# sdbds/ACE-Step-1.5-for-windows

Measured on AMD Instinct MI355X. Metric: songs/sec (30 s audio @ 27 DiT steps, CFG 7 + APG, batch 8 in total, DiT + VAE decode), higher is better.
Workload: dtype bf16; 1 GPU; acestep-5Hz base DiT (24L/2048d, 1.575B params, random init) + Oobleck decoder, 30 s audio (T=750), 27 steps, CFG 7 (2x8 sequences/forward on rank 0), L=769, 8 songs per request over 1 GPU(s); infer_steps=27, batch_per_gpu=8, batch_rank0=8, global_batch=8, parallelism=dp1, tiny=False, sampler_chains_per_gpu=1, batch_dependent_bits=True

## Files before the change

### ace-step-1.5-for-windows_amd/csrc/common.h

```cpp
#pragma once
#include <hip/hip_runtime.h>
#include <stdint.h>
#include <string>

namespace ace355 {

void set_error(const std::string& msg);
int hip_fail(hipError_t e, const char* what, const char* file, int line);

#define ACE_HIP(expr)                                                          \
    do {                                                                       \
        hipError_t _e = (expr);                                                \
        if (_e != hipSuccess) return ::ace355::hip_fail(_e, #expr, __FILE__, __LINE__); \
    } while (0)

#define ACE_CHECK(cond, msg)                                  \
    do {                                                      \
        if (!(cond)) {                                        \
            ::ace355::set_error(std::string("invalid argument: ") + (msg)); \
            return 1;                                         \
        }                                                     \
    } while (0)

#define ACE_LAUNCH_CHECK() ACE_HIP(hipGetLastError())
// ... 182 lines not shown
int launch_latent_check(const float* x, long n, int* flags_dev, hipStream_t s);
int launch_zero_u64(unsigned long long* p, long n, hipStream_t s);

enum PackMode { PACK_ROWS = 0, PACK_ROWS_IL32 = 1, PACK_CONV_IN = 2, PACK_CONVT_OUT = 3, PACK_ROWS_HEADPAIR = 4 };
__host__ __device__ __forceinline__ long pack_row(int mode, long r, long dst_row0, int p0) {
    if (mode == PACK_ROWS_IL32) return dst_row0 + (r >> 5) * 64 + p0 * 32 + (r & 31);
    if (mode == PACK_ROWS_HEADPAIR) {
        const long d = r & 127;
        return dst_row0 + (r - d) + (d < 64 ? 2 * d : 2 * (d - 64) + 1);
    }
    return dst_row0 + r;
}
int launch_pack(const void* src, int src_dtype, void* dst, int dst_is_bf16, int mode, long rows, long cols, long dst_ld,
                long dst_row0, int p0, int p1, hipStream_t s);

struct ConvArgs {
    const bf16_t* x; long x_batch_stride; int L_in; int Cin;
    long x_shift; long x_valid;
    const bf16_t* w;
    const float* bias;
    const float* alpha; const float* beta;
    const bf16_t* res; long res_batch_stride;
    void* y; long y_batch_stride;
    int B, M, N, taps, dil, center;
    long y_shift; long y_valid;
    int out_mode;
    int n_real;
    long ncl_ld; long ncl_off; int ncl_m_lo; int ncl_m_hi;
    int wide_ok;
    int clk_probe;
    const bf16_t* w2; const float* bias2; const float* alpha2; const float* beta2;
    const float* osnake_a; const float* osnake_b;
    int ras_tm; int ras_tn;
};
int launch_conv(const ConvArgs& a, hipStream_t s);
int launch_ncl_to_nlc(const float* z, bf16_t* out, int B, int C, int T, hipStream_t s);

constexpr int LORA_TILE_ROWS = 64, LORA_TILE_COLS = 128;
struct LoraTermDev {
    const bf16_t* A;
    const bf16_t* B;
    int rank;
    float scale;
};
struct LoraTargetDev {
    bf16_t* dst;
    const bf16_t* src;
    long ld;
    long row0;
    int mode, p0;
    int rows, cols;
    int tile0, tiles_n;
    int term0, nterms;
};
int launch_lora_merge(const LoraTargetDev* targets_dev, int n_targets, int total_tiles, const LoraTermDev* terms_dev, hipStream_t s);
int launch_lora_read(const bf16_t* w, long ld, int mode, long row0, int p0, long rows, long cols, void* dst, int dst_is_bf16,
                     hipStream_t s);

constexpr int XATTN_MAX_HEADS = 64;
struct XattnArgs {
    const bf16_t* q; long q_seq_stride; int q_ld;
    unsigned long long k_tab[64]; int k_ld;
    float* out;
    int N, Sq, Skv, Hq, Hkv, n_heads;
    int heads[XATTN_MAX_HEADS];
    float scale;
// ... 5 lines not shown
```

### ace-step-1.5-for-windows_amd/csrc/conv.hip

```cpp
#include <stdio.h>
#include <stdlib.h>

#include "common.h"


namespace ace355 {

namespace {

__device__ __forceinline__ int lds_off(int row, int slot) { return row * 128 + ((slot ^ ((row >> 1) & 7)) << 4); }

__device__ unsigned long long g_conv_probe[8];

typedef unsigned int u32x4 __attribute__((ext_vector_type(4)));
__device__ __forceinline__ u32x4 ld_u32x4(const void* p) {
    return *reinterpret_cast<const __attribute__((address_space(1))) u32x4*>(reinterpret_cast<uintptr_t>(p));
}

__device__ __forceinline__ void conv_glds16_v(const void* vptr, unsigned lds_addr) {
    unsigned keep;
    asm volatile("s_mov_b32 %0, m0\n\ts_mov_b32 m0, %2\n\ts_nop 0\n\tglobal_load_lds_dwordx4 %1, off\n\ts_mov_b32 m0, %0"
                 : "=&s"(keep)
                 : "v"(vptr), "s"(lds_addr)
                 : "memory");
}

constexpr int HALO_MAX = 64;

__device__ __forceinline__ void conv_glds16(unsigned voff, const void* sbase, unsigned lds_addr) {
    unsigned keep;
    asm volatile("s_mov_b32 %0, m0\n\ts_mov_b32 m0, %3\n\ts_nop 0\n\tglobal_load_lds_dwordx4 %1, %2\n\ts_mov_b32 m0, %0"
                 : "=&s"(keep)
                 : "v"(voff), "s"(sbase), "s"(lds_addr)
                 : "memory");
}

__device__ __forceinline__ bf16x8 frag_kperm(const char* base, int row, int q, int h) {
    const uint2 lo = *reinterpret_cast<const uint2*>(base + lds_off(row, 2 * q) + 8 * h);
    const uint2 hi = *reinterpret_cast<const uint2*>(base + lds_off(row, 2 * q + 1) + 8 * h);
    return as_bf16x8(make_uint4(lo.x, lo.y, hi.x, hi.y));
}

template <int BN, int TM, int WS = 0>
__global__ __launch_bounds__(TM * 2, TM / 64) void conv_kernel(ConvArgs a) {
    static_assert(TM == 128 || (TM == 256 && BN == 128), "tile shapes");
    static_assert(WS == 0 || (TM == 256 && BN == 128), "the 32 x 128 wave shape belongs to the fused 8-wave form");
    constexpr int NTHR = TM * 2;
    constexpr int WIN_MAX = TM + HALO_MAX;
    constexpr int MT = WS ? 1 : ((BN == 128) ? 2 : 1);
    constexpr int NT = WS ? 4 : ((BN == 128) ? 2 : 1);
    constexpr int WCH = BN * 8 / NTHR;
    constexpr int FUSE_LDS = (BN == 128 && TM == 128) ? (BN * 128 + 2048) : (WS ? 2048 : 0);
    __shared__ __attribute__((aligned(16))) char smem[WIN_MAX * 128 + 2 * BN * 128 + FUSE_LDS];
    char* As = smem;
    char* Wbase = smem + WIN_MAX * 128;

    const int tid = threadIdx.x, lane = tid & 63, wave = tid >> 6;
    const int lq = lane & 31, half = lane >> 5;
    const int wm = WS ? wave : ((BN == 128) ? (wave >> 1) : wave);
    const int wn = WS ? 0 : ((BN == 128) ? (wave & 1) : 0);
    int bx = blockIdx.x, by = blockIdx.y;
    if (a.ras_tn > 1) {
        const int L = blockIdx.x, tn = a.ras_tn, full = (a.ras_tm >> 3) << 3;
        if (L < full * tn) {
            const int q = L >> 3;
            by = q % tn;
            bx = (q / tn) * 8 + (L & 7);
        } else {
            const int l2 = L - full * tn;
            by = l2 % tn;
            bx = full + l2 / tn;
        }
    }
    const int m0 = bx * TM, n0 = by * BN, b = blockIdx.z;
    const int Cin = a.Cin, taps = a.taps, dil = a.dil;
    const int win_rows = TM + (taps - 1) * dil;
    const int x_row0 = m0 - a.center * dil;
    const bf16_t* xb = a.x + (long)b * a.x_batch_stride;
    const long wrow = (long)taps * Cin;

    f32x16 acc[MT][NT];
#pragma unroll
    for (int i = 0; i < MT; ++i)
#pragma unroll
        for (int j = 0; j < NT; ++j)
#pragma unroll
            for (int r = 0; r < 16; ++r) acc[i][j][r] = 0.f;

    const int sslot = tid & 7;
    constexpr int NWV = NTHR / 64;
    static_assert(WCH * NWV * 8 == BN, "pieces split evenly over the waves");
    unsigned w_voff[WCH];
    int wst[WCH];
#pragma unroll
    for (int i = 0; i < WCH; ++i) {
        const int prow = 8 * (wave + NWV * i) + (lane >> 3);
        const int ls = (lane & 7) ^ ((prow >> 1) & 7);
        w_voff[i] = (unsigned)(((long)min(n0 + prow, a.N - 1) * wrow + ls * 8) * 2);
        wst[i] = lds_off((tid >> 3) + (NTHR / 8) * i, sslot);
    }
    const unsigned wlds0 = (unsigned)(uintptr_t)Wbase + (unsigned)__builtin_amdgcn_readfirstlane(wave) * 1024u;
    auto w_piece = [&](int i, int tap, int ci0, int buf) {
        const bf16_t* sb = a.w + (long)tap * Cin + ci0;
        const unsigned lb = (unsigned)__builtin_amdgcn_readfirstlane((int)(wlds0 + (unsigned)buf * (BN * 128)));
        conv_glds16(w_voff[i], sb, lb + (unsigned)i * (NWV * 1024));
    };
    auto w_issue = [&](int tap, int ci0, int buf) {
// ... 88 lines not shown
        for (int i = 0; i < WLD; ++i) {
            const int c = tid + i * NTHR;
            if (c < win_rows * 8) *reinterpret_cast<u32x4*>(As + st0 + i * (NTHR / 8) * 128) = wv[i];
        }
    };
    const bool probe = a.clk_probe && blockIdx.x == gridDim.x / 2 && blockIdx.y == 0 && blockIdx.z == 0 && __builtin_amdgcn_readfirstlane(wave) == 0;
    unsigned long long p_t0 = 0, p_w0 = 0, p_stage = 0, p_taps = 0, p_mark = 0;
    if (probe) p_t0 = clock64(), p_w0 = wall_clock64();
    constexpr bool FPIPE = (TM == 128);
    if (PREFETCH) { win_load(0); if (PARPRE) par_load(0); }
    for (int ci0 = 0; ci0 < Cin; ci0 += 64) {
        if (probe) p_mark = clock64();
        if (!PREFETCH) win_load(ci0);
        __syncthreads();
        if (PREFETCH) __builtin_amdgcn_s_waitcnt(0x0F70);
        w_issue(0, ci0, 0);
        win_store(ci0);
        asm volatile("s_waitcnt vmcnt(0)" ::: "memory");
        __syncthreads();
        if (PREFETCH && ci0 + 64 < Cin) { win_load(ci0 + 64); if (PARPRE) par_load(ci0 + 64); }
        if (probe) { const unsigned long long t = clock64(); p_stage += t - p_mark; p_mark = t; }

#pragma unroll 1
        for (int tap = 0; tap < taps; ++tap) {
            const bool more = (tap + 1) < taps;
            if (more) w_issue(tap + 1, ci0, (tap + 1) & 1);
            if constexpr (FUSE_LDS != 0) {
                if (a.w2 && ci0 + 64 >= Cin) {
                    constexpr int PT_OFF = (WS ? 2 : 3) * BN * 128;
                    if constexpr (WS == 0) {
                        const unsigned w2b = (unsigned)(uintptr_t)(Wbase + 2 * BN * 128) + (unsigned)__builtin_amdgcn_readfirstlane(wave) * 1024u;
                        if (tap >= 1 && tap <= WCH) w2_piece(tap - 1, 0, w2b);
                    }
                    if (tap == 5 && __builtin_amdgcn_readfirstlane(wave) < 2) {
                        const float* src = (wave == 0) ? (lane < 32 ? (a.bias ? a.bias : a.alpha2) : a.alpha2)
                                                       : (lane < 32 ? a.beta2 : (a.bias2 ? a.bias2 : a.beta2));
                        conv_glds16_v(src + 4 * (lane & 31), (unsigned)(uintptr_t)(Wbase + PT_OFF) + (unsigned)__builtin_amdgcn_readfirstlane(wave) * 1024u);
                    }
                    if (!more) {
                        const unsigned ring = wlds0 + (unsigned)((tap + 1) & 1) * (BN * 128);
#pragma unroll
                        for (int i = 0; i < WCH; ++i) w2_piece(i, WS ? 0 : 1, ring);
                    }
                }
            }
            const char* Ws = Wbase + (tap & 1) * (BN * 128);
            const int arow = wm * (MT * 32) + tap * dil + lq;
            if constexpr (FPIPE) {
                bf16x8 fa[2][MT], fw[2][NT];
                auto frag = [&](int kk, int sl) {
#pragma unroll
                    for (int i = 0; i < MT; ++i)
                        fa[sl][i] = as_bf16x8(*reinterpret_cast<const uint4*>(As + lds_off(arow + i * 32, kk * 2 + half)));
#pragma unroll
                    for (int j = 0; j < NT; ++j)
                        fw[sl][j] = as_bf16x8(*reinterpret_cast<const uint4*>(Ws + lds_off(wn * (NT * 32) + j * 32 + lq, kk * 2 + half)));
                };
                frag(0, 0);
#pragma unroll
                for (int kk = 0; kk < 4; ++kk) {
                    if (kk < 3) frag(kk + 1, (kk + 1) & 1);
                    __builtin_amdgcn_sched_barrier(0);
#pragma unroll
                    for (int i = 0; i < MT; ++i)
#pragma unroll
                        for (int j = 0; j < NT; ++j) acc[i][j] = mfma32(fw[kk & 1][j], fa[kk & 1][i], acc[i][j]);
                    __builtin_amdgcn_sched_barrier(0);
                }
            } else {
#pragma unroll
                for (int kk = 0; kk < 4; ++kk) {
                    bf16x8 fa[MT], fw[NT];
#pragma unroll
                    for (int i = 0; i < MT; ++i)
                        fa[i] = as_bf16x8(*reinterpret_cast<const uint4*>(As + lds_off(arow + i * 32, kk * 2 + half)));
#pragma unroll
                    for (int j = 0; j < NT; ++j)
                        fw[j] = as_bf16x8(*reinterpret_cast<const uint4*>(Ws + lds_off(wn * (NT * 32) + j * 32 + lq, kk * 2 + half)));
#pragma unroll
                    for (int i = 0; i < MT; ++i)
#pragma unroll
                        for (int j = 0; j < NT; ++j) acc[i][j] = mfma32(fw[j], fa[i], acc[i][j]);
                }
            }
            if (more) {
                asm volatile("s_waitcnt vmcnt(0)" ::: "memory");
                __syncthreads();
            }
        }
        if (probe) p_taps += clock64() - p_mark;
    }
    const bool full = (m0 + TM <= a.M) && (n0 + BN <= a.N) &&
                      ((long)m0 * a.N + n0 + a.y_shift >= 0) && ((long)(m0 + TM - 1) * a.N + n0 + BN - 1 + a.y_shift < a.y_valid);
    const bool wide = BN == 128 && a.out_mode == 0 && full && a.wide_ok;
    const int mw0 = m0 + wm * (MT * 32), nw0 = n0 + wn * (NT * 32);
    const int row_l = lane >> 2, c4 = lane & 3;
    u32x4 bl[NT], bh[NT];
    u32x4 rv[2][MT * 2];
    const bool has_res = (TM == 128 || WS == 1) && a.res != nullptr;
    auto res_load = [&](int j, u32x4 (&r)[MT * 2]) {
        const long rcol = (long)b * a.res_batch_stride + nw0 + j * 32 + c4 * 8 + a.y_shift;
#pragma unroll
        for (int t = 0; t < MT * 2; ++t) r[t] = ld_u32x4(a.res + rcol + (long)(mw0 + t * 16 + row_l) * a.N);
    };
    auto epi_pre = [&](const float* eb) {
#pragma unroll
        for (int j = 0; j < NT; ++j) {
            bl[j] = u32x4{0u, 0u, 0u, 0u};
            bh[j] = u32x4{0u, 0u, 0u, 0u};
        }
        if (eb && WS == 0) {
#pragma unroll
            for (int j = 0; j < NT; ++j) {
                bl[j] = ld_u32x4(eb + nw0 + j * 32 + c4 * 8);
                bh[j] = ld_u32x4(eb + nw0 + j * 32 + c4 * 8 + 4);
            }
        }
        if (has_res) res_load(0, rv[0]);
    };
    bool epi_pre_done = false;
    const float* epi_bias = a.bias;
    bool bias_in_lds = false;
    if constexpr (WS == 1) {
        if (a.w2) {
            epi_bias = a.bias2;
            bias_in_lds = a.bias2 != nullptr;
            const float b7s = a.bias ? 1.f : 0.f;
            const char* W2c0 = Wbase + (taps & 1) * (BN * 128);
            const char* W2c1 = Wbase + ((taps + 1) & 1) * (BN * 128);
            const char* Pt = Wbase + 2 * BN * 128;
            __syncthreads();
            {
                const unsigned ring = wlds0 + (unsigned)(taps & 1 ? 0 : 1) * (BN * 128);
#pragma unroll
                for (int i = 0; i < WCH; ++i) w2_piece(i, 1, ring);
            }
// ... 86 lines not shown
                    const char* Ap = A2 + (k8 >> 2) * 16384;
                    const char* Wp = (k8 >> 2) ? W2c1 : W2c0;
                    const int kk = k8 & 3;
#pragma unroll
                    for (int i = 0; i < MT; ++i) fa[sl][i] = frag_kperm(Ap, wm * (MT * 32) + i * 32 + lq, kk, half);
#pragma unroll
                    for (int j = 0; j < NT; ++j) fw[sl][j] = frag_kperm(Wp, wn * (NT * 32) + j * 32 + lq, kk, half);
                };
                frag2(0, 0);
#pragma unroll
                for (int k8 = 0; k8 < 8; ++k8) {
                    if (k8 < 7) frag2(k8 + 1, (k8 + 1) & 1);
                    __builtin_amdgcn_sched_barrier(0);
#pragma unroll
                    for (int i = 0; i < MT; ++i)
#pragma unroll
                        for (int j = 0; j < NT; ++j) acc[i][j] = mfma32(fw[k8 & 1][j], fa[k8 & 1][i], acc[i][j]);
                    __builtin_amdgcn_sched_barrier(0);
                }
            }
        }
    }
    const unsigned long long p_e0 = probe ? clock64() : 0ull;
    auto probe_done = [&]() {
        if (!probe) return;
        __builtin_amdgcn_s_waitcnt(0x0F70);
        const unsigned long long t = clock64();
        g_conv_probe[0] = t - p_t0, g_conv_probe[1] = p_stage, g_conv_probe[2] = p_taps, g_conv_probe[3] = t - p_e0;
        g_conv_probe[4] = wall_clock64() - p_w0, g_conv_probe[5] = (unsigned long long)(Cin / 64);
    };

    if (wide) {
        if (!epi_pre_done) epi_pre(epi_bias);
        __syncthreads();
        char* stg = smem + wave * (MT * 32 * 128);
#pragma unroll
        for (int j = 0; j < NT; ++j) {
#pragma unroll
            for (int i = 0; i < MT; ++i)
#pragma unroll
                for (int g = 0; g < 4; ++g) {
                    float4 v;
                    v.x = acc[i][j][4 * g + 0]; v.y = acc[i][j][4 * g + 1]; v.z = acc[i][j][4 * g + 2]; v.w = acc[i][j][4 * g + 3];
                    const int row = i * 32 + lq, slot = 2 * g + half;
                    *reinterpret_cast<float4*>(stg + row * 128 + ((slot ^ (row & 7)) << 4)) = v;
                }
            if (has_res && j + 1 < NT) res_load(j + 1, rv[(j + 1) & 1]);
            u32x4 oa[2], ob[2];
            if (a.osnake_a) {
#pragma unroll
                for (int q = 0; q < 2; ++q) {
                    oa[q] = ld_u32x4(a.osnake_a + nw0 + j * 32 + c4 * 8 + 4 * q);
                    ob[q] = ld_u32x4(a.osnake_b + nw0 + j * 32 + c4 * 8 + 4 * q);
                }
            }
            const long col = (long)b * a.y_batch_stride + nw0 + j * 32 + c4 * 8 + a.y_shift;
            if constexpr (WS == 1) {
                if (bias_in_lds) {
                    const char* pb = Wbase + 2 * BN * 128 + 1536 + (nw0 + j * 32 + c4 * 8) * 4;
                    bl[j] = *reinterpret_cast<const u32x4*>(pb);
                    bh[j] = *reinterpret_cast<const u32x4*>(pb + 16);
                } else if (epi_bias) {
                    bl[j] = ld_u32x4(epi_bias + nw0 + j * 32 + c4 * 8);
                    bh[j] = ld_u32x4(epi_bias + nw0 + j * 32 + c4 * 8 + 4);
                }
            }
            const float bias[8] = {__uint_as_float(bl[j][0]), __uint_as_float(bl[j][1]), __uint_as_float(bl[j][2]), __uint_as_float(bl[j][3]),
                                   __uint_as_float(bh[j][0]), __uint_as_float(bh[j][1]), __uint_as_float(bh[j][2]), __uint_as_float(bh[j][3])};
#pragma unroll
            for (int t = 0; t < MT * 2; ++t) {
                const int row = t * 16 + row_l;
                const float4 lo = *reinterpret_cast<const float4*>(stg + row * 128 + (((2 * c4) ^ (row & 7)) << 4));
                const float4 hi = *reinterpret_cast<const float4*>(stg + row * 128 + (((2 * c4 + 1) ^ (row & 7)) << 4));
                float v[8] = {lo.x + bias[0], lo.y + bias[1], lo.z + bias[2], lo.w + bias[3],
                              hi.x + bias[4], hi.y + bias[5], hi.z + bias[6], hi.w + bias[7]};
                if (has_res) {
                    const u32x4 r = rv[j & 1][t];
#pragma unroll
                    for (int e2 = 0; e2 < 4; ++e2) { v[2 * e2] += bf_lo(r[e2]); v[2 * e2 + 1] += bf_hi(r[e2]); }
                }
                if (a.osnake_a) {
#pragma unroll
                    for (int e = 0; e < 8; ++e) {
                        const float sn = __sinf(__uint_as_float(oa[e >> 2][e & 3]) * v[e]);
                        v[e] = v[e] + __uint_as_float(ob[e >> 2][e & 3]) * sn * sn;
                    }
                }
                u32x4 pk = {pack_bf2(v[0], v[1]), pack_bf2(v[2], v[3]), pack_bf2(v[4], v[5]), pack_bf2(v[6], v[7])};
                *reinterpret_cast<u32x4*>(reinterpret_cast<bf16_t*>(a.y) + col + (long)(mw0 + row) * a.N) = pk;
            }
        }
        probe_done();
        return;
    }
#pragma unroll
    for (int i = 0; i < MT; ++i) {
        const int m = mw0 + i * 32 + lq;
        if (m >= a.M) continue;
#pragma unroll
        for (int j = 0; j < NT; ++j)
#pragma unroll
            for (int r = 0; r < 16; ++r) {
                const int n = nw0 + j * 32 + 8 * (r >> 2) + 4 * half + (r & 3);
                if (n >= a.N) continue;
                float v = acc[i][j][r] + (epi_bias ? epi_bias[n] : 0.f);
                if (a.out_mode == 0) {
                    const long flat = (long)m * a.N + n + a.y_shift;
                    if (flat < 0 || flat >= a.y_valid) continue;
                    if (a.res) v += bf2f(a.res[(long)b * a.res_batch_stride + flat]);
                    if (a.osnake_a) {
                        const float sn = __sinf(a.osnake_a[n] * v);
                        v = v + a.osnake_b[n] * sn * sn;
                    }
                    reinterpret_cast<bf16_t*>(a.y)[(long)b * a.y_batch_stride + flat] = f2bf(v);
                } else {
                    if (n < a.n_real) {
                        if (a.ncl_ld == 0) reinterpret_cast<float*>(a.y)[(long)b * a.y_batch_stride + (long)n * a.M + m] = v;
                        else if (m >= a.ncl_m_lo && m < a.ncl_m_hi)
                            reinterpret_cast<float*>(a.y)[(long)b * a.y_batch_stride + (long)n * a.ncl_ld + a.ncl_off + (m - a.ncl_m_lo)] = v;
                    }
                }
            }
    }
}

__global__ void ncl_to_nlc_kernel(const float* __restrict__ z, bf16_t* __restrict__ out, int C, int T, long total) {
    const long i = (long)blockIdx.x * blockDim.x + threadIdx.x;
    if (i >= total) return;
    const int c = (int)(i % C);
    const long bt = i / C;
    const int t = (int)(bt % T);
    const long b = bt / T;
    out[i] = f2bf(z[(b * C + c) * T + t]);
}

}

int launch_conv(const ConvArgs& a, hipStream_t s) {
    ACE_CHECK(a.Cin % 64 == 0, "conv: Cin must be a multiple of 64");
    ACE_CHECK(a.taps >= 1 && (a.taps - 1) * a.dil <= HALO_MAX && a.dil >= 1, "conv: window too large");
    ACE_CHECK(a.B > 0 && a.M > 0 && a.N > 0, "conv: empty problem");
    ACE_CHECK((long)a.N * a.taps * a.Cin * 2 < (1L << 32) && (reinterpret_cast<uintptr_t>(a.w) & 15) == 0,
              "conv: the weight tensor must be 16-byte aligned and smaller than 4 GB (32-bit DMA offsets)");
    ACE_CHECK(a.x_valid ? (a.x_shift % 8 == 0 && a.x_valid % 8 == 0) : a.x_shift == 0, "conv: x_shift / x_valid must be multiples of 8 (and x_shift needs x_valid)");
    ACE_CHECK(!a.w2 || (a.Cin == 128 && a.N == 128 && a.taps == 7 && !a.x_valid && a.out_mode == 0 && a.alpha2 && a.beta2 &&
                        (reinterpret_cast<uintptr_t>(a.alpha2) & 15) == 0 && (reinterpret_cast<uintptr_t>(a.beta2) & 15) == 0 &&
                        (reinterpret_cast<uintptr_t>(a.bias) & 15) == 0 && (reinterpret_cast<uintptr_t>(a.w2) & 15) == 0),
              "conv: the fused k = 1 stage needs Cin = N = 128, a plain conv and 16-byte aligned vectors");
    ACE_CHECK(!a.osnake_a == !a.osnake_b && (!a.osnake_a || a.out_mode == 0), "conv: the producer-side Snake needs both parameter vectors and the bf16 output");
    ConvArgs aw = a;
    {
        auto al16 = [](const void* p) { return (reinterpret_cast<uintptr_t>(p) & 15) == 0; };
        aw.wide_ok = a.out_mode == 0 && al16(a.y) && al16(a.res) && al16(a.bias) && al16(a.bias2) && al16(a.osnake_a) && al16(a.osnake_b) &&
                     (a.N % 8) == 0 && (a.y_shift % 8) == 0 &&
                     (a.y_batch_stride % 8) == 0 && (a.res_batch_stride % 8) == 0;
    }
    static int tm_env = -1, clk_env = -1, ras_env = -1;
    if (ras_env < 0) {
        const char* e = getenv("ACE355_CONV_RAS");
        ras_env = e ? atoi(e) : 1;
    }
    if (clk_env < 0) {
        const char* e = getenv("ACE355_CONV_CLK");
        clk_env = e ? atoi(e) : 0;
    }
    aw.clk_probe = clk_env;
    if (tm_env < 0) {
        const char* e = getenv("ACE355_CONV_TM");
        tm_env = e ? atoi(e) : 0;
    }
    if (a.N >= 128 || a.N % 128 == 0) {
        const long wgs128 = (long)((a.M + 127) / 128) * ((a.N + 127) / 128) * a.B;
        const bool tall_k = a.Cin >= 128 && a.taps >= 3 && wgs128 >= 1400;
        const bool tall_t = a.taps == 2 && a.Cin >= 128 && !a.alpha && !a.x_valid && wgs128 >= 1500;
        const bool tall = !a.w2 && !a.res && (tm_env ? tm_env == 256 : (tall_k || tall_t));
        const int tm_rows = tall ? 256 : 128;
        dim3 grid((a.M + tm_rows - 1) / tm_rows, (a.N + 127) / 128, a.B);
        aw.ras_tm = aw.ras_tn = 0;
        if (ras_env && grid.y > 1 && (long)grid.x * grid.y < (1L << 31)) {
            aw.ras_tm = (int)grid.x, aw.ras_tn = (int)grid.y;
            grid = dim3(grid.x * grid.y, 1, a.B);
        }
        static int f8_env = -2;
        if (f8_env == -2) {
            const char* e = getenv("ACE355_CONV_F8");
            f8_env = e ? atoi(e) : -1;
        }
        const bool f8 = a.w2 && (f8_env >= 0 ? f8_env != 0 : wgs128 >= 1400);
        if (f8) {
            dim3 g8((a.M + 255) / 256, 1, a.B);
            aw.ras_tm = aw.ras_tn = 0;
            hipLaunchKernelGGL((conv_kernel<128, 256, 1>), g8, dim3(512), 0, s, aw);
        } else
        if (tall) hipLaunchKernelGGL((conv_kernel<128, 256>), grid, dim3(512), 0, s, aw);
        else hipLaunchKernelGGL((conv_kernel<128, 128>), grid, dim3(256), 0, s, aw);
    } else {
        aw.ras_tm = aw.ras_tn = 0;
        dim3 grid((a.M + 127) / 128, (a.N + 31) / 32, a.B);
        hipLaunchKernelGGL((conv_kernel<32, 128>), grid, dim3(256), 0, s, aw);
    }
    ACE_LAUNCH_CHECK();
    if (aw.clk_probe) {
        ACE_HIP(hipStreamSynchronize(s));
        unsigned long long h[8];
        ACE_HIP(hipMemcpyFromSymbol(h, HIP_SYMBOL(g_conv_probe), sizeof(h)));
        fprintf(stderr, "[conv clk] Cin=%d N=%d taps=%d dil=%d M=%d: total %llu cyc = stage %llu + taps %llu + epilogue %llu (+%llu other), wall %.2f us, %llu chunks\n",
                a.Cin, a.N, a.taps, a.dil, a.M, h[0], h[1], h[2], h[3], h[0] - h[1] - h[2] - h[3], h[4] / 100.0, h[5]);
    }
    return 0;
}

int launch_ncl_to_nlc(const float* z, bf16_t* out, int B, int C, int T, hipStream_t s) {
    const long total = (long)B * C * T;
    hipLaunchKernelGGL(ncl_to_nlc_kernel, dim3((unsigned)((total + 255) / 256)), dim3(256), 0, s, z, out, C, T, total);
    ACE_LAUNCH_CHECK();
    return 0;
}

}
```

### ace-step-1.5-for-windows_amd/csrc/vae.hip

```cpp
#include <math.h>
#include <string.h>

#include <algorithm>
#include <map>
#include <string>
#include <vector>

#include "../../include/ace355.h"
#include "common.h"

using namespace ace355;

namespace {

struct ConvW {
    bf16_t* w = nullptr;
    float* bias = nullptr;
    int N = 0, taps = 0, Cin = 0;
};
struct SnakeP {
    float* ea = nullptr;
    float* ib = nullptr;
};
struct ResUnitW {
// ... 300 lines not shown
    c->bias = b->p;
    ACE_LAUNCH_CHECK();
    return 0;
}

int build_snake_tiled(ace355_vae* h, const std::string& base, int C, int reps, SnakeP* sp) {
    SnakeP one;
    int rc = build_snake(h, base, C, &one);
    if (rc) return rc;
    if ((rc = valloc(h, &sp->ea, (size_t)C * reps))) return rc;
    if ((rc = valloc(h, &sp->ib, (size_t)C * reps))) return rc;
    hipLaunchKernelGGL(tile_bias_kernel, dim3((C * reps + 255) / 256), dim3(256), 0, 0, one.ea, sp->ea, C, reps);
    hipLaunchKernelGGL(tile_bias_kernel, dim3((C * reps + 255) / 256), dim3(256), 0, 0, one.ib, sp->ib, C, reps);
    ACE_LAUNCH_CHECK();
    return 0;
}

int build_res_unit(ace355_vae* h, const std::string& r, int C, int dil, ResUnitW* R) {
    int rc;
    R->dil = dil;
    if ((rc = build_snake(h, r + ".snake1", C, &R->s1))) return rc;
    if ((rc = build_conv(h, r + ".conv1", C, C, 7, true, &R->c1))) return rc;
    if ((rc = build_snake(h, r + ".snake2", C, &R->s2))) return rc;
    return build_conv(h, r + ".conv2", C, C, 1, true, &R->c2);
}

int run_conv(ace355_vae* h, const ConvArgs& a, hipStream_t s) {
    hipEvent_t e0 = nullptr, e1 = nullptr;
    if (h->profile) {
        hipEventCreate(&e0); hipEventCreate(&e1);
        hipEventRecord(e0, s);
        h->flops += 2.0 * a.B * (double)a.M * (a.out_mode == 1 ? a.n_real : a.N) * a.taps * a.Cin;
        if (a.w2) h->flops += 2.0 * a.B * (double)a.M * a.N * a.N;
        h->launches++;
    }
    int rc = launch_conv(a, s);
    if (h->profile) {
        hipEventRecord(e1, s);
        h->ev.push_back({e0, e1});
    }
    return rc;
}

}

extern "C" {

int ace355_vae_create(const ace355_vae_config* cfg, ace355_vae** out) {
    ACE_CHECK(cfg && out, "vae_create: null argument");
    ACE_CHECK(cfg->num_blocks > 0 && cfg->num_blocks <= ACE355_MAX_BLOCKS, "vae_create: num_blocks");
    ACE_CHECK(cfg->decoder_input_channels % 64 == 0 && cfg->decoder_channels % 64 == 0, "vae_create: channels must be multiples of 64");
    ACE_CHECK(cfg->audio_channels >= 1 && cfg->audio_channels <= 32, "vae_create: audio_channels");
    ace355_vae* h = new ace355_vae();
    h->cfg = *cfg;
    h->hop = 1;
    for (int i = 0; i < cfg->num_blocks; ++i) {
        ACE_CHECK(cfg->upsampling_ratios[i] >= 1 && cfg->channel_multiples[i] >= 1, "vae_create: ratios/multiples");
        h->hop *= cfg->upsampling_ratios[i];
    }
    if (const char* e = getenv("ACE355_VAE_BUDGET_MB")) { const long mb = atol(e); if (mb > 0) h->decode_budget = (size_t)mb << 20; }
    *out = h;
    return ACE355_OK;
}

void ace355_vae_destroy(ace355_vae* h) {
    if (!h) return;
// ... 92 lines not shown
        }
        if ((rc = build_snake(h, "encoder.snake1", EH * cm[nb], &h->e_s_out))) return rc;
        if ((rc = build_conv(h, "encoder.conv2", EH, EH * cm[nb], 3, true, &h->e_conv2))) return rc;
    }
    ACE_HIP(hipDeviceSynchronize());
    for (auto& kv : h->raw) {
        const std::string& k = kv.first;
        const bool keep = k.size() > 5 && k.compare(k.size() - 5, 5, ".bias") == 0;
        if (!keep && kv.second.p) { hipFree(kv.second.p); kv.second.p = nullptr; }
    }
    if (!h->scratch) ACE_HIP(hipMalloc((void**)&h->scratch, 1024));
    h->finalized = true;
    return ACE355_OK;
}

int ace355_vae_hop(const ace355_vae* h) { return h ? h->hop : 0; }

static int episnake_on() {
    static int on = -1;
    if (on < 0) {
        const char* e = getenv("ACE355_VAE_EPISNAKE");
        on = e ? atoi(e) : 1;
    }
    return on;
}
static bool unit_fused(int C) {
    static int fuse = -1;
    if (fuse < 0) {
        const char* e = getenv("ACE355_CONV_FUSE_RU");
        fuse = e ? atoi(e) : 1;
    }
    return fuse && C == 128;
}

static void stage_push(std::vector<ace355_vae_stage_info>& v, int kind, int block, int unit, int channels, int flags, int src, int res,
                       int dil, long rows) {
    ace355_vae_stage_info si;
    si.kind = kind; si.block = block; si.unit = unit; si.channels = channels; si.flags = flags; si.src = src; si.res = res;
    si.dilation = dil; si.rows = rows;
    v.push_back(si);
}
static void stage_push_unit(std::vector<ace355_vae_stage_info>& v, int block, int unit, int C, int dil, long rows, bool epi, bool out_snake) {
    const int in = (int)v.size() - 1;
    const int osn = out_snake ? ACE355_VAE_FLAG_OUT_SNAKE : 0;
    if (unit_fused(C)) {
        stage_push(v, ACE355_VAE_STAGE_UNIT, block, unit, C, ACE355_VAE_FLAG_FUSED | ACE355_VAE_FLAG_IN_SNAKE | osn, in, in, dil, rows);
        return;
    }
    stage_push(v, ACE355_VAE_STAGE_UNIT_K7, block, unit, C, ACE355_VAE_FLAG_IN_SNAKE | (epi ? ACE355_VAE_FLAG_OUT_SNAKE : 0), in, -1, dil, rows);
    stage_push(v, ACE355_VAE_STAGE_UNIT_K1, block, unit, C, (epi ? 0 : ACE355_VAE_FLAG_IN_SNAKE) | osn, in + 1, in, 1, rows);
}
static int stage_list(const ace355_vae* h, int enc, long T, std::vector<ace355_vae_stage_info>& v) {
    v.clear();
    const ace355_vae_config& c = h->cfg;
    if (!enc) {
        const bool epi = episnake_on() != 0 && !h->blocks.empty();
        stage_push(v, ACE355_VAE_STAGE_INPUT, -1, -1, c.decoder_input_channels, 0, -1, -1, 1, T);
        stage_push(v, ACE355_VAE_STAGE_CONV_IN, -1, -1, h->conv1.N, epi ? ACE355_VAE_FLAG_OUT_SNAKE : 0, 0, -1, 1, T);
        long L = T;
        for (size_t bi = 0; bi < h->blocks.size(); ++bi) {
            const BlockW& Bk = h->blocks[bi];
            L = (L - 1) * Bk.stride - 2 * Bk.pad + 2 * Bk.stride;
            stage_push(v, ACE355_VAE_STAGE_CONVT, (int)bi, -1, Bk.cout, epi ? 0 : ACE355_VAE_FLAG_IN_SNAKE, (int)v.size() - 1, -1, 1, L);
            for (int j = 0; j < 3; ++j) stage_push_unit(v, (int)bi, j, Bk.cout, Bk.ru[j].dil, L, epi, epi && j == 2);
        }
        return 0;
// ... 19 lines not shown
static int tap_stage(ace355_vae* h, int enc, int kind, const void* p, int B, hipStream_t s) {
    if (h->tap_stages.empty()) return 0;
    const int k = h->tap_next++;
    ACE_CHECK(k < (int)h->tap_stages.size() && h->tap_stages[k].kind == kind, "vae tap: the stage list and the launch sequence disagree");
    auto it = h->taps[enc].find(k);
    if (it == h->taps[enc].end()) return 0;
    const ace355_vae_stage_info& si = h->tap_stages[k];
    const size_t bytes = (size_t)B * si.rows * si.channels * ((si.flags & ACE355_VAE_FLAG_F32_NCL) ? 4 : 2);
    ACE_CHECK(bytes <= it->second.second, "vae tap: the destination is smaller than the stage");
    ACE_HIP(hipMemcpyAsync(it->second.first, p, bytes, hipMemcpyDeviceToDevice, s));
    return 0;
}
static int tap_begin(ace355_vae* h, int enc, long T, bool single_window) {
    h->tap_stages.clear();
    h->tap_next = 0;
    if (h->taps[enc].empty()) return 0;
    if (!single_window) {
        set_error("vae tap: the call splits into several windows under the activation budget; a tap needs one whole-sequence window");
        return ACE355_ERR_STATE;
    }
    int rc = stage_list(h, enc, T, h->tap_stages);
    if (rc) { h->tap_stages.clear(); return rc; }
    ACE_CHECK(h->taps[enc].rbegin()->first < (int)h->tap_stages.size(), "vae tap: no such stage");
    return 0;
}
static int tap_end(ace355_vae* h) {
    const bool ok = h->tap_stages.empty() || h->tap_next == (int)h->tap_stages.size();
    h->tap_stages.clear();
    ACE_CHECK(ok, "vae tap: the stage list and the launch sequence disagree");
    return 0;
}

static int run_res_unit(ace355_vae* h, const ResUnitW& R, bf16_t*& state, bf16_t*& tmp, int B, long L, int C, hipStream_t s,
                        int enc, const SnakeP* out_snake = nullptr) {
    if (unit_fused(C)) {
        ConvArgs f{};
        f.x = state; f.x_batch_stride = L * C; f.L_in = (int)L; f.Cin = C;
        f.w = R.c1.w; f.bias = R.c1.bias; f.alpha = R.s1.ea; f.beta = R.s1.ib;
        f.w2 = R.c2.w; f.bias2 = R.c2.bias; f.alpha2 = R.s2.ea; f.beta2 = R.s2.ib;
        f.res = state; f.res_batch_stride = L * C;
        f.y = tmp; f.y_batch_stride = L * C;
        f.B = B; f.M = (int)L; f.N = C; f.taps = 7; f.dil = R.dil; f.center = 3;
        f.y_shift = 0; f.y_valid = L * C; f.out_mode = 0;
        if (out_snake) f.osnake_a = out_snake->ea, f.osnake_b = out_snake->ib;
        const int rcf = run_conv(h, f, s);
        if (rcf) return rcf;
        std::swap(state, tmp);
        return tap_stage(h, enc, ACE355_VAE_STAGE_UNIT, state, B, s);
    }
    ConvArgs a{};
    a.x = state; a.x_batch_stride = L * C; a.L_in = (int)L; a.Cin = C;
    a.w = R.c1.w; a.bias = R.c1.bias; a.alpha = R.s1.ea; a.beta = R.s1.ib;
    a.y = tmp; a.y_batch_stride = L * C;
    a.B = B; a.M = (int)L; a.N = C; a.taps = 7; a.dil = R.dil; a.center = 3;
    a.y_shift = 0; a.y_valid = L * C; a.out_mode = 0;
    const bool epi = episnake_on() != 0;
    if (epi) a.osnake_a = R.s2.ea, a.osnake_b = R.s2.ib;
    int rc = run_conv(h, a, s);
    if (rc) return rc;
    if ((rc = tap_stage(h, enc, ACE355_VAE_STAGE_UNIT_K7, tmp, B, s))) return rc;
    a = ConvArgs{};
    a.x = tmp; a.x_batch_stride = L * C; a.L_in = (int)L; a.Cin = C;
    a.w = R.c2.w; a.bias = R.c2.bias;
    if (!epi) a.alpha = R.s2.ea, a.beta = R.s2.ib;
    if (out_snake) a.osnake_a = out_snake->ea, a.osnake_b = out_snake->ib;
    a.res = state; a.res_batch_stride = L * C;
    a.y = state; a.y_batch_stride = L * C;
    a.B = B; a.M = (int)L; a.N = C; a.taps = 1; a.dil = 1; a.center = 0;
    a.y_shift = 0; a.y_valid = L * C; a.out_mode = 0;
    if ((rc = run_conv(h, a, s))) return rc;
    return tap_stage(h, enc, ACE355_VAE_STAGE_UNIT_K1, state, B, s);
}

static size_t decode_elems(const ace355_vae* h, long frames) {
    size_t need = (size_t)frames * h->conv1.N;
    long L = frames;
    for (const BlockW& Bk : h->blocks) {
// ... 3 lines not shown
    return need;
}
static size_t decode_bytes(const ace355_vae* h, int nb, long frames) { return 3 * (decode_elems(h, frames) * (size_t)nb * 2 + 256); }

static int decode_receptive_frames(const ace355_vae* h) {
    double rf = 3.0, rate = 1.0;
    for (const BlockW& Bk : h->blocks) {
        rf += 1.0 / rate;
        rate *= Bk.stride;
        rf += 3.0 * (1 + 3 + 9) / rate;
    }
    rf += 3.0 / rate;
    return (int)ceil(rf);
}

static int decode_window(ace355_vae* h, int b0, int nb, int T, int ws, int we, int cs, int ce, float* wav_out_dev, hipStream_t s) {
    const ace355_vae_config& c = h->cfg;
    const int Tw = we - ws;
    bf16_t *cur = h->buf[0], *nxt = h->buf[1], *tmp = h->buf[2];
    long L = Tw;
    int rc;
    ConvArgs a{};
    a.x = h->zin + ((size_t)b0 * T + ws) * c.decoder_input_channels; a.x_batch_stride = (long)T * c.decoder_input_channels; a.L_in = Tw;
    a.Cin = c.decoder_input_channels;
    a.w = h->conv1.w; a.bias = h->conv1.bias;
    a.y = cur; a.y_batch_stride = (long)Tw * h->conv1.N;
    a.B = nb; a.M = Tw; a.N = h->conv1.N; a.taps = 7; a.dil = 1; a.center = 3;
    a.y_shift = 0; a.y_valid = (long)Tw * h->conv1.N; a.out_mode = 0;
    const bool epi = episnake_on() != 0 && !h->blocks.empty();
    if (epi) a.osnake_a = h->blocks[0].s1.ea, a.osnake_b = h->blocks[0].s1.ib;
    if ((rc = run_conv(h, a, s))) return rc;
    if ((rc = tap_stage(h, 0, ACE355_VAE_STAGE_CONV_IN, cur, nb, s))) return rc;

    for (size_t bi = 0; bi < h->blocks.size(); ++bi) {
        const BlockW& Bk = h->blocks[bi];
        const SnakeP* next_snake = !epi ? nullptr : (bi + 1 < h->blocks.size() ? &h->blocks[bi + 1].s1 : &h->s_out);
        const long Lout = (L - 1) * Bk.stride - 2 * Bk.pad + 2 * Bk.stride;
        a = ConvArgs{};
        a.x = cur; a.x_batch_stride = L * Bk.cin; a.L_in = (int)L; a.Cin = Bk.cin;
        a.w = Bk.ct.w; a.bias = Bk.ct.bias;
        if (!epi) a.alpha = Bk.s1.ea, a.beta = Bk.s1.ib;
        a.y = nxt; a.y_batch_stride = Lout * Bk.cout;
        a.B = nb; a.M = (int)L + 1; a.N = Bk.ct.N; a.taps = 2; a.dil = 1; a.center = 1;
        a.y_shift = -(long)Bk.pad * Bk.cout; a.y_valid = Lout * Bk.cout; a.out_mode = 0;
        if ((rc = run_conv(h, a, s))) return rc;
        if ((rc = tap_stage(h, 0, ACE355_VAE_STAGE_CONVT, nxt, nb, s))) return rc;
        for (int j = 0; j < 3; ++j)
            if ((rc = run_res_unit(h, Bk.ru[j], nxt, tmp, nb, Lout, Bk.cout, s, 0, j == 2 ? next_snake : nullptr))) return rc;
        std::swap(cur, nxt);
        L = Lout;
    }
    const long hop = h->hop, Lall = hop * T;
    a = ConvArgs{};
    a.x = cur; a.x_batch_stride = L * c.decoder_channels; a.L_in = (int)L; a.Cin = c.decoder_channels;
    a.w = h->conv2.w; a.bias = nullptr;
    if (!epi) a.alpha = h->s_out.ea, a.beta = h->s_out.ib;
    a.y = wav_out_dev + (size_t)b0 * c.audio_channels * Lall; a.y_batch_stride = Lall * c.audio_channels;
    a.B = nb; a.M = (int)L; a.N = c.audio_channels; a.taps = 7; a.dil = 1; a.center = 3;
    a.out_mode = 1; a.n_real = c.audio_channels;
    a.ncl_ld = Lall; a.ncl_off = (long)cs * hop; a.ncl_m_lo = (int)((cs - ws) * hop); a.ncl_m_hi = (int)((ce - ws) * hop);
    return run_conv(h, a, s);
}

static int decode_plan(const ace355_vae* h, int B, int T, size_t budget, int* nb_out, int* tc_out, int* ov_out) {
    const int rf = decode_receptive_frames(h);
    int ov = h->decode_overlap > 0 ? h->decode_overlap : std::max(16, ((rf + 2 + 7) / 8) * 8);
    ACE_CHECK(ov >= rf, "vae_decode: the window overlap must cover the decoder's receptive field");
    int nb = B, tc = T;
    if (decode_bytes(h, B, T) > budget) {
        const size_t per_item = decode_bytes(h, 1, T);
        if (per_item <= budget) nb = (int)std::max<size_t>(1, std::min<size_t>(B, budget / per_item));
        else {
            nb = 1;
            const size_t per_frame = decode_bytes(h, 1, 1024) / 1024 + 1;
            const long win = (long)(budget / per_frame);
            tc = (int)std::min<long>(T, win - 2L * ov);
            ACE_CHECK(tc >= ov, "vae_decode: the activation budget is smaller than one decode window (raise ACE355_VAE_BUDGET_MB)");
            tc = (tc / 8) * 8;
            const size_t per_win = decode_bytes(h, 1, std::min<long>(T, tc + 2L * ov));
            nb = (int)std::max<size_t>(1, std::min<size_t>(B, budget / per_win));
        }
    }
    *nb_out = nb; *tc_out = tc; *ov_out = ov;
    return 0;
}

int ace355_vae_decode(ace355_vae* h, const float* z_dev, int B, int T, float* wav_out_dev, void* stream) {
    RoctxRange r_dec("ace355.vae_decode");
    ACE_CHECK(h && z_dev && wav_out_dev, "vae_decode: null argument");
    if (!h->finalized) { set_error("vae_decode: call ace355_vae_finalize first"); return ACE355_ERR_STATE; }
    ACE_CHECK(B > 0 && T > 0, "vae_decode: empty problem");
    ACE_CHECK((long)T * h->hop < (1L << 31), "vae_decode: sequence too long (2^31 samples per item)");
    hipStream_t s = (hipStream_t)stream;
// ... 249 lines not shown
```

Measured before the change: 17.09 songs/s.

## Fold the VAE output conv into the last fused residual-unit kernel

The final 7-tap output convolution (128 to 2 channels) now runs inside the epilogue of the last fused residual-unit conv kernel. Snake-activated tiles are staged in LDS with a 3-row halo and reduced with MFMA straight to the float waveform. This removes one launch and the write and re-read of the largest full-resolution bf16 activation. In exchange, tiles overlap by 6 rows so edge rows are recomputed, and the epilogue uses more LDS. The fold is on by default and can be disabled with an environment variable.

```diff
diff --git a/ace-step-1.5-for-windows_amd/csrc/common.h b/ace-step-1.5-for-windows_amd/csrc/common.h
--- a/ace-step-1.5-for-windows_amd/csrc/common.h
+++ b/ace-step-1.5-for-windows_amd/csrc/common.h
@@ -238,6 +238,7 @@
     const bf16_t* w2; const float* bias2; const float* alpha2; const float* beta2;
     const float* osnake_a; const float* osnake_b;
     int ras_tm; int ras_tn;
+    const bf16_t* fold_w; float* fold_y; long fold_y_batch_stride;
 };
 int launch_conv(const ConvArgs& a, hipStream_t s);
 int launch_ncl_to_nlc(const float* z, bf16_t* out, int B, int C, int T, hipStream_t s);
diff --git a/ace-step-1.5-for-windows_amd/csrc/conv.hip b/ace-step-1.5-for-windows_amd/csrc/conv.hip
--- a/ace-step-1.5-for-windows_amd/csrc/conv.hip
+++ b/ace-step-1.5-for-windows_amd/csrc/conv.hip
@@ -41,16 +41,17 @@
     return as_bf16x8(make_uint4(lo.x, lo.y, hi.x, hi.y));
 }
 
-template <int BN, int TM, int WS = 0>
+template <int BN, int TM, int WS = 0, int FOLD = 0>
 __global__ __launch_bounds__(TM * 2, TM / 64) void conv_kernel(ConvArgs a) {
     static_assert(TM == 128 || (TM == 256 && BN == 128), "tile shapes");
     static_assert(WS == 0 || (TM == 256 && BN == 128), "the 32 x 128 wave shape belongs to the fused 8-wave form");
+    static_assert(FOLD == 0 || (BN == 128 && (WS == 1 || TM == 128)), "the folded output conv belongs to the one-launch unit forms");
     constexpr int NTHR = TM * 2;
     constexpr int WIN_MAX = TM + HALO_MAX;
     constexpr int MT = WS ? 1 : ((BN == 128) ? 2 : 1);
     constexpr int NT = WS ? 4 : ((BN == 128) ? 2 : 1);
     constexpr int WCH = BN * 8 / NTHR;
-    constexpr int FUSE_LDS = (BN == 128 && TM == 128) ? (BN * 128 + 2048) : (WS ? 2048 : 0);
+    constexpr int FUSE_LDS = (BN == 128 && TM == 128) ? (BN * 128 + 2048) : (WS ? (FOLD ? 3072 : 2048) : 0);
     __shared__ __attribute__((aligned(16))) char smem[WIN_MAX * 128 + 2 * BN * 128 + FUSE_LDS];
     char* As = smem;
     char* Wbase = smem + WIN_MAX * 128;
@@ -72,7 +73,7 @@
             bx = full + l2 / tn;
         }
     }
-    const int m0 = bx * TM, n0 = by * BN, b = blockIdx.z;
+    const int m0 = FOLD ? bx * (TM - 6) - 3 : bx * TM, n0 = by * BN, b = blockIdx.z;
     const int Cin = a.Cin, taps = a.taps, dil = a.dil;
     const int win_rows = TM + (taps - 1) * dil;
     const int x_row0 = m0 - a.center * dil;
@@ -227,9 +228,12 @@
                         const unsigned w2b = (unsigned)(uintptr_t)(Wbase + 2 * BN * 128) + (unsigned)__builtin_amdgcn_readfirstlane(wave) * 1024u;
                         if (tap >= 1 && tap <= WCH) w2_piece(tap - 1, 0, w2b);
                     }
-                    if (tap == 5 && __builtin_amdgcn_readfirstlane(wave) < 2) {
+                    if (tap == 5 && __builtin_amdgcn_readfirstlane(wave) < ((FOLD && WS) ? 3 : 2)) {
                         const float* src = (wave == 0) ? (lane < 32 ? (a.bias ? a.bias : a.alpha2) : a.alpha2)
                                                        : (lane < 32 ? a.beta2 : (a.bias2 ? a.bias2 : a.beta2));
+                        if constexpr (FOLD && WS) {
+                            if (wave == 2) src = lane < 32 ? a.osnake_a : a.osnake_b;
+                        }
                         conv_glds16_v(src + 4 * (lane & 31), (unsigned)(uintptr_t)(Wbase + PT_OFF) + (unsigned)__builtin_amdgcn_readfirstlane(wave) * 1024u);
                     }
                     if (!more) {
@@ -287,7 +291,7 @@
     }
     const bool full = (m0 + TM <= a.M) && (n0 + BN <= a.N) &&
                       ((long)m0 * a.N + n0 + a.y_shift >= 0) && ((long)(m0 + TM - 1) * a.N + n0 + BN - 1 + a.y_shift < a.y_valid);
-    const bool wide = BN == 128 && a.out_mode == 0 && full && a.wide_ok;
+    const bool wide = FOLD ? true : (BN == 128 && a.out_mode == 0 && full && a.wide_ok);
     const int mw0 = m0 + wm * (MT * 32), nw0 = n0 + wn * (NT * 32);
     const int row_l = lane >> 2, c4 = lane & 3;
     u32x4 bl[NT], bh[NT];
@@ -296,7 +300,10 @@
     auto res_load = [&](int j, u32x4 (&r)[MT * 2]) {
         const long rcol = (long)b * a.res_batch_stride + nw0 + j * 32 + c4 * 8 + a.y_shift;
 #pragma unroll
-        for (int t = 0; t < MT * 2; ++t) r[t] = ld_u32x4(a.res + rcol + (long)(mw0 + t * 16 + row_l) * a.N);
+        for (int t = 0; t < MT * 2; ++t) {
+            if constexpr (FOLD) r[t] = ld_u32x4(a.res + rcol + (long)min(max(mw0 + t * 16 + row_l, 0), a.M - 1) * a.N);
+            else r[t] = ld_u32x4(a.res + rcol + (long)(mw0 + t * 16 + row_l) * a.N);
+        }
     };
     auto epi_pre = [&](const float* eb) {
 #pragma unroll
@@ -449,7 +456,16 @@
 
     if (wide) {
         if (!epi_pre_done) epi_pre(epi_bias);
+        constexpr int FS_OFF = 32768, FW_OFF = 65536;
+        int tf = tid;
+        if constexpr (FOLD) asm volatile("" : "+v"(tf));
+        const int f_wave = __builtin_amdgcn_readfirstlane(tf >> 6), f_lq = tf & 31, f_half = (tf >> 5) & 1, f_rowl = (tf & 63) >> 2, f_c4 = tf & 3;
+        u32x4 fhold[2];
         __syncthreads();
+        if constexpr (FOLD) {
+            if (f_wave < 4)
+                conv_glds16_v(a.fold_w + min(tf, a.n_real * 112 - 1) * 8, (unsigned)(uintptr_t)(smem + FW_OFF) + (unsigned)f_wave * 1024u);
+        }
         char* stg = smem + wave * (MT * 32 * 128);
 #pragma unroll
         for (int j = 0; j < NT; ++j) {
@@ -464,6 +480,14 @@
                 }
             if (has_res && j + 1 < NT) res_load(j + 1, rv[(j + 1) & 1]);
             u32x4 oa[2], ob[2];
+            if constexpr (FOLD && WS == 1) {
+                const char* po = Wbase + 2 * BN * 128 + 2048 + (j * 32 + c4 * 8) * 4;
+#pragma unroll
+                for (int q = 0; q < 2; ++q) {
+                    oa[q] = *reinterpret_cast<const u32x4*>(po + 16 * q);
+                    ob[q] = *reinterpret_cast<const u32x4*>(po + 512 + 16 * q);
+                }
+            } else
             if (a.osnake_a) {
 #pragma unroll
                 for (int q = 0; q < 2; ++q) {
@@ -504,12 +528,65 @@
                     }
                 }
                 u32x4 pk = {pack_bf2(v[0], v[1]), pack_bf2(v[2], v[3]), pack_bf2(v[4], v[5]), pack_bf2(v[6], v[7])};
-                *reinterpret_cast<u32x4*>(reinterpret_cast<bf16_t*>(a.y) + col + (long)(mw0 + row) * a.N) = pk;
+                if constexpr (FOLD) {
+                    if ((unsigned)(mw0 + row) >= (unsigned)a.M) pk = u32x4{0u, 0u, 0u, 0u};
+                    const int f_wm = WS ? f_wave : (f_wave >> 1), f_wn = WS ? 0 : (f_wave & 1);
+                    const int srow = f_wm * (MT * 32) + t * 16 + f_rowl;
+                    const int ch8 = f_wn * (NT * 4) + j * 4 + f_c4;
+                    if constexpr (WS == 1) {
+                        if (j < 2) *reinterpret_cast<u32x4*>(smem + FS_OFF + lds_off(srow, ch8)) = pk;
+                        else if (j == 2) fhold[t & 1] = pk;
+                        else {
+                            *reinterpret_cast<u32x4*>(smem + lds_off(srow, f_c4)) = fhold[t & 1];
+                            *reinterpret_cast<u32x4*>(smem + lds_off(srow, 4 + f_c4)) = pk;
+                        }
+                    } else {
+                        *reinterpret_cast<u32x4*>(smem + FS_OFF + (ch8 >> 3) * (TM * 128) + lds_off(srow, ch8 & 7)) = pk;
+                    }
+                } else {
+                    *reinterpret_cast<u32x4*>(reinterpret_cast<bf16_t*>(a.y) + col + (long)(mw0 + row) * a.N) = pk;
+                }
+            }
+        }
+        if constexpr (FOLD) {
+            asm volatile("s_waitcnt vmcnt(0)" ::: "memory");
+            __syncthreads();
+            const char* Sp0 = smem + FS_OFF;
+            const char* Sp1 = WS ? smem : smem + FS_OFF + TM * 128;
+            const char* Fw = smem + FW_OFF + min(f_lq, a.n_real - 1) * (7 * 256) + f_half * 16;
+            f32x16 z;
+#pragma unroll
+            for (int r = 0; r < 16; ++r) z[r] = 0.f;
+#pragma unroll
+            for (int c = 0; c < 2; ++c) {
+                const char* Sp = c ? Sp1 : Sp0;
+#pragma unroll 1
+                for (int tap = 0; tap < 7; ++tap) {
+                    const int srow = min(max(f_wave * 32 + f_lq + tap - 3, 0), TM - 1);
+#pragma unroll
+                    for (int kk = 0; kk < 4; ++kk) {
+                        const bf16x8 fa = as_bf16x8(*reinterpret_cast<const uint4*>(Sp + lds_off(srow, kk * 2 + f_half)));
+                        const bf16x8 fw = as_bf16x8(*reinterpret_cast<const uint4*>(Fw + tap * 256 + c * 128 + kk * 32));
+                        z = mfma32(fw, fa, z);
+                    }
+                }
+            }
+            const int r_t = f_wave * 32 + f_lq, m = m0 + r_t;
+            if (f_half == 0 && r_t >= 3 && r_t < TM - 3 && m < a.M) {
+                float* yo = a.fold_y + (long)b * a.fold_y_batch_stride;
+#pragma unroll
+                for (int n = 0; n < 2; ++n) {
+                    if (n >= a.n_real) continue;
+                    const float v = z[n] + 0.f;
+                    if (a.ncl_ld == 0) yo[(long)n * a.M + m] = v;
+                    else if (m >= a.ncl_m_lo && m < a.ncl_m_hi) yo[(long)n * a.ncl_ld + a.ncl_off + (m - a.ncl_m_lo)] = v;
+                }
             }
         }
         probe_done();
         return;
     }
+    if constexpr (FOLD) return;
 #pragma unroll
     for (int i = 0; i < MT; ++i) {
         const int m = mw0 + i * 32 + lq;
@@ -565,6 +642,8 @@
                         (reinterpret_cast<uintptr_t>(a.bias) & 15) == 0 && (reinterpret_cast<uintptr_t>(a.w2) & 15) == 0),
               "conv: the fused k = 1 stage needs Cin = N = 128, a plain conv and 16-byte aligned vectors");
     ACE_CHECK(!a.osnake_a == !a.osnake_b && (!a.osnake_a || a.out_mode == 0), "conv: the producer-side Snake needs both parameter vectors and the bf16 output");
+    ACE_CHECK(!a.fold_w || (a.w2 && a.res && a.osnake_a && a.fold_y && a.n_real >= 1 && a.n_real <= 2 && (reinterpret_cast<uintptr_t>(a.fold_w) & 15) == 0),
+              "conv: the folded output conv needs the one-launch unit with a residual and the reader's Snake, and at most 2 output channels");
     ConvArgs aw = a;
     {
         auto al16 = [](const void* p) { return (reinterpret_cast<uintptr_t>(p) & 15) == 0; };
@@ -604,6 +683,12 @@
             f8_env = e ? atoi(e) : -1;
         }
         const bool f8 = a.w2 && (f8_env >= 0 ? f8_env != 0 : wgs128 >= 1400);
+        if (a.fold_w) {
+            ACE_CHECK(aw.wide_ok, "conv: the folded output conv needs 16-byte aligned activations");
+            aw.ras_tm = aw.ras_tn = 0;
+            if (f8) hipLaunchKernelGGL((conv_kernel<128, 256, 1, 1>), dim3((a.M + 249) / 250, 1, a.B), dim3(512), 0, s, aw);
+            else hipLaunchKernelGGL((conv_kernel<128, 128, 0, 1>), dim3((a.M + 121) / 122, 1, a.B), dim3(256), 0, s, aw);
+        } else
         if (f8) {
             dim3 g8((a.M + 255) / 256, 1, a.B);
             aw.ras_tm = aw.ras_tn = 0;
diff --git a/ace-step-1.5-for-windows_amd/csrc/vae.hip b/ace-step-1.5-for-windows_amd/csrc/vae.hip
--- a/ace-step-1.5-for-windows_amd/csrc/vae.hip
+++ b/ace-step-1.5-for-windows_amd/csrc/vae.hip
@@ -356,6 +356,7 @@
         hipEventRecord(e0, s);
         h->flops += 2.0 * a.B * (double)a.M * (a.out_mode == 1 ? a.n_real : a.N) * a.taps * a.Cin;
         if (a.w2) h->flops += 2.0 * a.B * (double)a.M * a.N * a.N;
+        if (a.fold_w) h->flops += 2.0 * a.B * (double)a.M * a.n_real * 7 * a.N;
         h->launches++;
     }
     int rc = launch_conv(a, s);
@@ -514,6 +515,14 @@
     }
     return fuse && C == 128;
 }
+static bool fold_out_on() {
+    static int on = -1;
+    if (on < 0) {
+        const char* e = getenv("ACE355_CONV_FOLD_OUT");
+        on = e ? atoi(e) : 1;
+    }
+    return on != 0;
+}
 
 static void stage_push(std::vector<ace355_vae_stage_info>& v, int kind, int block, int unit, int channels, int flags, int src, int res,
                        int dil, long rows) {
@@ -599,7 +608,7 @@
 }
 
 static int run_res_unit(ace355_vae* h, const ResUnitW& R, bf16_t*& state, bf16_t*& tmp, int B, long L, int C, hipStream_t s,
-                        int enc, const SnakeP* out_snake = nullptr) {
+                        int enc, const SnakeP* out_snake = nullptr, const ConvArgs* fold_out = nullptr) {
     if (unit_fused(C)) {
         ConvArgs f{};
         f.x = state; f.x_batch_stride = L * C; f.L_in = (int)L; f.Cin = C;
@@ -610,6 +619,11 @@
         f.B = B; f.M = (int)L; f.N = C; f.taps = 7; f.dil = R.dil; f.center = 3;
         f.y_shift = 0; f.y_valid = L * C; f.out_mode = 0;
         if (out_snake) f.osnake_a = out_snake->ea, f.osnake_b = out_snake->ib;
+        if (fold_out) {
+            f.fold_w = fold_out->w; f.fold_y = reinterpret_cast<float*>(fold_out->y); f.fold_y_batch_stride = fold_out->y_batch_stride;
+            f.n_real = fold_out->n_real;
+            f.ncl_ld = fold_out->ncl_ld; f.ncl_off = fold_out->ncl_off; f.ncl_m_lo = fold_out->ncl_m_lo; f.ncl_m_hi = fold_out->ncl_m_hi;
+        }
         const int rcf = run_conv(h, f, s);
         if (rcf) return rcf;
         std::swap(state, tmp);
@@ -679,6 +693,14 @@
     if ((rc = run_conv(h, a, s))) return rc;
     if ((rc = tap_stage(h, 0, ACE355_VAE_STAGE_CONV_IN, cur, nb, s))) return rc;
 
+    const bool fold = fold_out_on() && epi && h->tap_stages.empty() && unit_fused(h->blocks.back().cout) &&
+                      h->conv2.Cin == h->blocks.back().cout && h->conv2.taps == 7 && c.audio_channels <= 2;
+    const long hop = h->hop, Lall = hop * T;
+    ConvArgs oc{};
+    oc.w = h->conv2.w;
+    oc.y = wav_out_dev + (size_t)b0 * c.audio_channels * Lall; oc.y_batch_stride = Lall * c.audio_channels;
+    oc.out_mode = 1; oc.n_real = c.audio_channels;
+    oc.ncl_ld = Lall; oc.ncl_off = (long)cs * hop; oc.ncl_m_lo = (int)((cs - ws) * hop); oc.ncl_m_hi = (int)((ce - ws) * hop);
     for (size_t bi = 0; bi < h->blocks.size(); ++bi) {
         const BlockW& Bk = h->blocks[bi];
         const SnakeP* next_snake = !epi ? nullptr : (bi + 1 < h->blocks.size() ? &h->blocks[bi + 1].s1 : &h->s_out);
@@ -693,19 +715,17 @@
         if ((rc = run_conv(h, a, s))) return rc;
         if ((rc = tap_stage(h, 0, ACE355_VAE_STAGE_CONVT, nxt, nb, s))) return rc;
         for (int j = 0; j < 3; ++j)
-            if ((rc = run_res_unit(h, Bk.ru[j], nxt, tmp, nb, Lout, Bk.cout, s, 0, j == 2 ? next_snake : nullptr))) return rc;
+            if ((rc = run_res_unit(h, Bk.ru[j], nxt, tmp, nb, Lout, Bk.cout, s, 0, j == 2 ? next_snake : nullptr,
+                                   (fold && j == 2 && bi + 1 == h->blocks.size()) ? &oc : nullptr))) return rc;
         std::swap(cur, nxt);
         L = Lout;
     }
-    const long hop = h->hop, Lall = hop * T;
-    a = ConvArgs{};
+    if (fold) return 0;
+    a = oc;
     a.x = cur; a.x_batch_stride = L * c.decoder_channels; a.L_in = (int)L; a.Cin = c.decoder_channels;
-    a.w = h->conv2.w; a.bias = nullptr;
+    a.bias = nullptr;
     if (!epi) a.alpha = h->s_out.ea, a.beta = h->s_out.ib;
-    a.y = wav_out_dev + (size_t)b0 * c.audio_channels * Lall; a.y_batch_stride = Lall * c.audio_channels;
     a.B = nb; a.M = (int)L; a.N = c.audio_channels; a.taps = 7; a.dil = 1; a.center = 3;
-    a.out_mode = 1; a.n_real = c.audio_channels;
-    a.ncl_ld = Lall; a.ncl_off = (long)cs * hop; a.ncl_m_lo = (int)((cs - ws) * hop); a.ncl_m_hi = (int)((ce - ws) * hop);
     return run_conv(h, a, s);
 }
 
```

New measurement: 17.07 songs/s, median of 2. No clear change (-0.2%).
